# LemonATsu/DANBO-pytorch

Measured on NVIDIA B200. Metric: DANBO render rays/s (fwd+composite), higher is better.
Workload: dtype bf16 (tensor-core MLP, fp32 accumulate); fp32 elsewhere; fp64 box test

## Files before the change

danbo-pytorch_b200/_lib.py:

```python
import ctypes
import os

_HERE = os.path.dirname(os.path.abspath(__file__))
_PATH = os.path.join(_HERE, "libdanbo_b200.so")
_lib = None
ABI_VERSION = 5

c_p = ctypes.c_void_p
c_i = ctypes.c_int
c_f = ctypes.c_float

_SIGNATURES = {
    "danbo_version": [],
    "danbo_nearfar": [c_p, c_i, c_i, c_p, c_i, c_p, c_i, c_i, c_p, c_p, c_i, c_i, c_f, c_f, c_p, c_p, c_p, c_i, c_p, c_p, c_p],
    "danbo_sample_mask": [c_p, c_i, c_i, c_i, c_p, c_p, c_p, c_p, c_p, c_p, c_p, c_i, c_i, c_p, c_p, c_p, c_p, c_i, c_i, c_i, c_p],
    "danbo_field_agg": [c_p, c_i, c_i, c_i, c_p, c_p, c_p, c_p, c_i, c_p, c_p, c_i, c_i, c_p, c_p, c_p, c_p, c_p, c_p, c_p, c_i, c_i, c_i, c_p],
    "danbo_agg_frag_bytes": [],
    "danbo_pair_logits_set_blocks": [c_i],
    "danbo_pack_agg_frags": [c_p, c_p, c_p],
    "danbo_ray_bias": [c_p, c_i, c_i, c_p, c_p, c_i, c_p, c_p, c_p, c_p],
    "danbo_mlp_workspace_bytes": [c_p, c_p, c_p],
    "danbo_mlp_set_pack_empty": [c_i],
    "danbo_mlp_empty_rows": [c_p, c_i, c_p, c_p, c_i, c_p],
    "danbo_mlp_set_cta_pair": [c_i],
    "danbo_graph_net_fwd": [c_p, c_i, c_p, c_p, c_p, c_p],
    "danbo_graph_net_bwd": [c_i, c_p, c_p, c_p, c_p, c_p, c_p],
    "danbo_graph_net_bwd_pose": [c_p, c_i, c_p, c_p, c_p, c_p, c_p],
    "danbo_pose_fwd": [c_p, c_p, c_p, c_p, c_p, c_i, c_p, c_p, c_i, c_i, c_p, c_p, c_f, c_f, c_f, c_p, c_p, c_p, c_p, c_p],
    "danbo_pose_bwd": [c_p, c_p, c_p, c_p, c_p, c_i, c_p, c_p, c_i, c_i, c_p, c_p, c_p, c_p, c_p, c_f, c_f, c_p, c_p, c_p,
                       c_p],
    "danbo_pose_kp2d": [c_p, c_p, c_p, c_i, c_f, c_f, c_p, c_p, c_p],
    "danbo_train_loss": [c_p, c_p, c_p, c_p, c_p, c_p, c_f, c_i, c_i, c_i, c_f, c_f, c_p, c_p, c_p, c_p, c_i, c_f, c_p, c_p, c_f,
                         c_p, c_p, c_p, c_p, c_p, c_p, c_p, c_p],
    "danbo_adam_step": [c_p, c_p, c_p, c_p, ctypes.c_longlong, c_p, c_f, c_f, c_f, c_p, c_i, c_p],
    "danbo_anerf_workspace_bytes": [c_i, c_p, c_p, c_p, c_p],
    "danbo_anerf_pack_weights": [c_p, c_p, c_p, c_p, c_p, c_p, c_p, c_p, c_p, c_p, c_p, c_p, c_p, c_p],
    "danbo_anerf_ray_encode": [c_p, c_i, c_i, c_p, c_i, c_i, c_p, c_p, c_i, c_p, c_p, c_p, c_p],
    "danbo_anerf_embed": [c_p, c_i, c_i, c_p, c_i, c_p, c_i, c_i, c_p, c_p, c_f, c_p, c_p, c_p],
    "danbo_anerf_mlp": [c_p, c_p, c_p, c_p, c_p, c_p, c_i, c_i, c_p, c_i, c_i, c_p, c_p],
    "danbo_anerf_save_bytes": [c_i, c_p],
    "danbo_anerf_mlp_save": [c_p, c_p, c_p, c_p, c_p, c_p, c_i, c_i, c_p, c_i, c_i, c_p, c_p],
# ... 23 lines not shown

EXPORTS = tuple(_SIGNATURES)


def path():
    return _PATH


def load():
    global _lib
    if _lib is None:
        if not os.path.exists(_PATH):
            raise RuntimeError(f"{_PATH} is missing: build it with `python __graft_entry__.py build` "
                               "(there is no CPU fallback for the DANBO hot path)")
        lib = ctypes.CDLL(_PATH)
        for name, argtypes in _SIGNATURES.items():
            fn = getattr(lib, name)
            fn.argtypes = argtypes
            fn.restype = ctypes.c_int
        got = lib.danbo_version()
        if got != ABI_VERSION:
            raise RuntimeError(f"{_PATH} has ABI version {got}, this binding expects {ABI_VERSION}: rebuild it with "
                               "`python __graft_entry__.py build`")
        if os.environ.get("DANBO_PAIR_LOGITS_BLOCKS", ""):
            lib.danbo_pair_logits_set_blocks(int(os.environ["DANBO_PAIR_LOGITS_BLOCKS"]))
        if os.environ.get("DANBO_MLP_CTA_PAIR", "") == "0":
            lib.danbo_mlp_set_cta_pair(0)
        _lib = lib
    return _lib


def check(code, what):
    if code != 0:
        raise RuntimeError(f"{what} failed with code {code}" + (" (cudaError)" if code > 0 else " (invalid argument)"))
```

danbo-pytorch_b200/csrc/field.cu:

```cuda
#include "field_common.cuh"

namespace danbo {

__global__ void nearfar_cyl_kernel(const float* __restrict__ rays, int ray_stride, int n_rays,
                                   const float* __restrict__ pose_cyl, int cyl_stride, int rays_per_pose, int n_poses,
                                   int seg_len, float* __restrict__ near_out, float* __restrict__ far_out,
                                   double* __restrict__ seg_acc ) {
    const int n = blockIdx.x * blockDim.x + threadIdx.x;
    if (n >= n_rays) return;
    const float* r = rays + (size_t)n * ray_stride;
    const float ox = r[0], oz = r[2], dx = r[3], dz = r[5], near = r[6], far = r[7];
    int pose = n / rays_per_pose; if (pose >= n_poses) pose = n_poses - 1;
    const float* c = pose_cyl + (size_t)pose * cyl_stride;
    const float cx = c[0], cz = c[1], rad = c[2];
    const float nx = __fadd_rn(ox, __fmul_rn(dx, near)), nz = __fadd_rn(oz, __fmul_rn(dz, near));
    const float fx = __fadd_rn(ox, __fmul_rn(dx, far)), fz = __fadd_rn(oz, __fmul_rn(dz, far));
    const float ncx = __fsub_rn(cx, nx), ncz = __fsub_rn(cz, nz);
    const float nfx = __fsub_rn(fx, nx), nfz = __fsub_rn(fz, nz);
    const float nf_norm = __fsqrt_rn(__fadd_rn(__fmul_rn(nfx, nfx), __fmul_rn(nfz, nfz)));
    const float scale = __fsqrt_rn(__fadd_rn(__fmul_rn(dx, dx), __fmul_rn(dz, dz)));
    const float cross = __fsub_rn(__fmul_rn(ncx, nfz), __fmul_rn(ncz, nfx));
    const float dist = __fdiv_rn(fabsf(cross), nf_norm);
    const float Q = __fsqrt_rn(__fsub_rn(__fmul_rn(rad, rad), __fmul_rn(dist, dist)));
    const float K = __fdiv_rn(__fadd_rn(__fmul_rn(ncx, nfx), __fmul_rn(ncz, nfz)), nf_norm);
// ... 455 lines not shown
#pragma unroll
                for (int o4 = 0; o4 < 4; ++o4) {
                    const float4 wv = __ldg(w1 + i * (DANBO_AGG_W / 4) + oh * 4 + o4);
#pragma unroll
                    for (int u = 0; u < PP; ++u) {
                        l1[u][4 * o4 + 0] = fmaf(mix[u][i], wv.x, l1[u][4 * o4 + 0]); l1[u][4 * o4 + 1] = fmaf(mix[u][i], wv.y, l1[u][4 * o4 + 1]);
                        l1[u][4 * o4 + 2] = fmaf(mix[u][i], wv.z, l1[u][4 * o4 + 2]); l1[u][4 * o4 + 3] = fmaf(mix[u][i], wv.w, l1[u][4 * o4 + 3]);
                    }
                }
            }
#pragma unroll
            for (int o = 0; o < 16; ++o) {
                const float w2 = __ldg(fc.agg_w2 + j * DANBO_AGG_W + oh * 16 + o);
#pragma unroll
                for (int u = 0; u < PP; ++u) a[u] = fmaf(fmaxf(l1[u][o], 0.f), w2, a[u]);
            }
        }
#pragma unroll
        for (int u = 0; u < PP; ++u)
            if (live[u]) logits[(size_t)id[u] * DANBO_J + j] = a[u];
    }
}

__global__ void __launch_bounds__(128)
field_rows_kernel(const float* __restrict__ rays, int ray_stride, int n_rays, int S, const float* __restrict__ z,
                  const uint32_t* __restrict__ mask, const int* __restrict__ active_ids,
                  const int* __restrict__ active_count, int capacity, const float* __restrict__ pose_skts,
                  const float* __restrict__ pose_vol, int rays_per_pose, int n_poses, FieldConsts fc,
                  const float* __restrict__ logits, uint8_t* __restrict__ xtiles, int* __restrict__ row_ray,
                  float* __restrict__ hbar_out ,
                  __nv_bfloat16* __restrict__ x_rows ,
                  int agg_mode , const int* __restrict__ work) {
    int count = *active_count; if (count > capacity) count = capacity;
    const int total = n_rays * S;
    const float poison = work[DANBO_PAIR_OVERFLOW_WORD] ? __int_as_float(0x7fc00000) : 0.f;
    __shared__ __align__(128) uint8_t stage[4][2][4096];
    const int warp = threadIdx.x >> 5, lane = threadIdx.x & 31;
    int n_flush = 0;
    for (int base = blockIdx.x * blockDim.x; base < count; base += gridDim.x * blockDim.x) {
        if (base + warp * 32 >= count) break;
        const int e = base + threadIdx.x;
        const bool live = e < count;
        const int id = live ? active_ids[e] : total;
        float hbar[DANBO_FEAT];
#pragma unroll
        for (int i = 0; i < DANBO_FEAT; ++i) hbar[i] = 0.f;
        int n;
// ... 32 lines not shown
        if (hbar_out && live) {
            float4* ho = reinterpret_cast<float4*>(hbar_out + (size_t)e * 16);
            ho[0] = make_float4(hbar[0], hbar[1], hbar[2], hbar[3]);   ho[1] = make_float4(hbar[4], hbar[5], hbar[6], hbar[7]);
            ho[2] = make_float4(hbar[8], hbar[9], hbar[10], hbar[11]); ho[3] = make_float4(hbar[12], hbar[13], hbar[14], 0.f);
        }
        float sn[DANBO_FEAT], cs[DANBO_FEAT];
#pragma unroll
        for (int i = 0; i < DANBO_FEAT; ++i) sincosf(hbar[i], &sn[i], &cs[i]);
        const int tile = e >> 7, rr = e & 127;
        uint8_t* xt = xtiles + (size_t)tile * DANBO_X_TILE_BYTES;
        uint32_t pk[4];
#pragma unroll
        for (int col = 0; col < 208; ++col) {
            float v;
            if (col < DANBO_FEAT) v = hbar[col];
            else if (col < DANBO_X_COLS) {
                const int q = col - DANBO_FEAT, rem = q % 30;
                v = rem < DANBO_FEAT ? sn[rem] : cs[rem - DANBO_FEAT];
            } else v = 0.f;
            const uint32_t b = __bfloat16_as_ushort(__float2bfloat16_rn(v));
            if (col & 1) pk[(col & 7) >> 1] |= b << 16; else pk[(col & 7) >> 1] = b;
            if ((col & 7) == 7) {
                const int chunk = (col - 7) >> 6, unit = ((col - 7) & 63) >> 3;
                if (unit == 0) {
                    if (n_flush >= 2) {
                        if (lane == 0) asm volatile("cp.async.bulk.wait_group.read 1;" ::: "memory");
                        __syncwarp();
                    }
                }
                const uint32_t dst = smem_u32(stage[warp][n_flush & 1]) + (uint32_t)(lane * 128 + ((unit ^ (lane & 7)) << 4));
                asm volatile("st.shared.v4.b32 [%0], {%1,%2,%3,%4};" ::"r"(dst), "r"(pk[0]), "r"(pk[1]), "r"(pk[2]), "r"(pk[3]) : "memory");
                if (x_rows && live) *reinterpret_cast<uint4*>(x_rows + (size_t)e * 208 + (col - 7)) = make_uint4(pk[0], pk[1], pk[2], pk[3]);
                if (unit == 7 || col == 207) {
                    asm volatile("fence.proxy.async.shared::cta;" ::: "memory");
                    __syncwarp();
                    if (lane == 0) {
                        uint8_t* gdst = xt + chunk * 16384 + warp * 4096;
                        asm volatile("cp.async.bulk.global.shared::cta.bulk_group [%0], [%1], %2;"
                                     ::"l"(gdst), "r"(smem_u32(stage[warp][n_flush & 1])), "r"(4096u) : "memory");
                        asm volatile("cp.async.bulk.commit_group;" ::: "memory");
                    }
                    ++n_flush;
                }
            }
            if (col >= 44 && (col - 44) % 30 == 0 && col < 194) {
#pragma unroll
                for (int i = 0; i < DANBO_FEAT; ++i) { const float s2 = 2.f * sn[i] * cs[i], c2 = 1.f - 2.f * sn[i] * sn[i]; sn[i] = s2; cs[i] = c2; }
            }
        }
    }
    if (lane == 0) asm volatile("cp.async.bulk.wait_group 0;" ::: "memory");
}

__global__ void __launch_bounds__(128)
code_table_kernel(const float* __restrict__ codes, const float* __restrict__ wv_ray, float* __restrict__ table) {
    const int ci = blockIdx.x, o = threadIdx.x;
    float acc = wv_ray[155 * 128 + o];
    for (int c = 0; c < 128; ++c) acc = fmaf(codes[(size_t)ci * 128 + c], wv_ray[(27 + c) * 128 + o], acc);
    table[ci * 128 + o] = acc;
}

__global__ void __launch_bounds__(128)
ray_bias_kernel(const float* __restrict__ rays, int ray_stride, int n_rays, const int* __restrict__ cam_idx, int n_codes,
                const float* __restrict__ wv_ray ,
                const float* __restrict__ table , float* __restrict__ out ) {
    constexpr int RB = 32, VIN = 27;
// ... 115 lines not shown
    const FieldConsts fc = make_consts(consts);
    const int total = n_rays * S;
    int blocks = (capacity + 255) / 256;
    if (blocks > num_sms * 8) blocks = num_sms * 8;
    pair_bucket_kernel<false><<<blocks, 256, 0, st>>>(mask, active_ids, active_count, capacity, total, pw, pair_capacity, agg_mode);
    DANBO_CHECK_LAUNCH();
    pair_bucket_kernel<true><<<blocks, 256, 0, st>>>(mask, active_ids, active_count, capacity, total, pw, pair_capacity, agg_mode);
    DANBO_CHECK_LAUNCH();
    int pblocks = (pair_capacity / 64 + 24 + 3) / 4;
    if (pblocks > num_sms * 8) pblocks = num_sms * 8;
    const void* agg_frags = consts[10];
    if (agg_frags != nullptr) {
        const int rc = launch_pair_logits_mma(rays, ray_stride, S, z, active_ids, pose_skts, pose_vol, rays_per_pose,
                                              n_poses, fc, pw, pair_capacity, agg_frags, logits, num_sms, st);
        if (rc != 0) return rc;
    } else if (n_poses == 1)
        pair_logits_kernel<true><<<pblocks, 128, 0, st>>>(rays, ray_stride, S, z, active_ids, pose_skts, pose_vol, rays_per_pose,
                                                           n_poses, fc, pw, pair_capacity, logits);
    else
        pair_logits_kernel<false><<<pblocks, 128, 0, st>>>(rays, ray_stride, S, z, active_ids, pose_skts, pose_vol, rays_per_pose,
                                                            n_poses, fc, pw, pair_capacity, logits);
    DANBO_CHECK_LAUNCH();
    int rblocks = (capacity + 127) / 128;
    if (rblocks > num_sms * 16) rblocks = num_sms * 16;
    field_rows_kernel<<<rblocks, 128, 0, st>>>(rays, ray_stride, n_rays, S, z, mask, active_ids, active_count, capacity,
                                                pose_skts, pose_vol, rays_per_pose, n_poses, fc, logits,
                                                (uint8_t*)xtiles, row_ray, hbar_out, (__nv_bfloat16*)x_rows, agg_mode, work);
    DANBO_CHECK_LAUNCH();
    return 0;
}

extern "C" int danbo_ray_bias(const float* rays, int ray_stride, int n_rays, const int* cam_idx, const float* codes,
                              int n_codes, const float* wv_ray, float* table, float* out, void* stream) {
    if (n_rays <= 0) return 0;
    if (!table) return -1;
    code_table_kernel<<<n_codes + 1, 128, 0, (cudaStream_t)stream>>>(codes, wv_ray, table);
    DANBO_CHECK_LAUNCH();
    ray_bias_kernel<<<(n_rays + 31) / 32, 128, 0, (cudaStream_t)stream>>>(rays, ray_stride, n_rays, cam_idx, n_codes, wv_ray,
                                                                       table, out);
    DANBO_CHECK_LAUNCH();
    return 0;
}
```

danbo-pytorch_b200/csrc/field_common.cuh:

```cuda
#pragma once
#include "common.cuh"
#include <math.h>

namespace danbo {

struct FieldConsts {
    const float* align;
    const float* axis_scale;
    const float* agg_w0;
    const float* agg_adjw;
    const float* agg_adj;
    const float* agg_b0;
    const float* agg_w1;
    const float* agg_b1;
    const float* agg_w2;
    const float* agg_b2;
};

static __constant__ uint32_t kNbrMask[DANBO_J] = {
    0x0000000Fu, 0x00000013u, 0x00000025u, 0x00000049u, 0x00000092u, 0x00000124u, 0x00000248u, 0x00000490u,
    0x00000920u, 0x00007240u, 0x00000480u, 0x00000900u, 0x00009200u, 0x00012200u, 0x00024200u, 0x00009000u,
    0x00052000u, 0x000A4000u, 0x00150000u, 0x002A0000u, 0x00540000u, 0x00A80000u, 0x00500000u, 0x00A00000u};

__device__ __forceinline__ void bone_aligned(const float* __restrict__ skt, const float* __restrict__ A,
// ... 12 lines not shown
    t2 = __fadd_rn(fmaf(a2.z, l2, fmaf(a2.y, l1, __fmul_rn(a2.x, l0))), a2.w);
}

__device__ __forceinline__ void bone_coords(const float* __restrict__ skt, const float* __restrict__ A,
                                            const float* __restrict__ scale, float px, float py, float pz,
                                            float& x0, float& x1, float& x2) {
    const float4 r0 = __ldg(reinterpret_cast<const float4*>(skt));
    const float4 r1 = __ldg(reinterpret_cast<const float4*>(skt) + 1);
    const float4 r2 = __ldg(reinterpret_cast<const float4*>(skt) + 2);
    const float l0 = fmaf(r0.z, pz, fmaf(r0.y, py, fmaf(r0.x, px, r0.w)));
    const float l1 = fmaf(r1.z, pz, fmaf(r1.y, py, fmaf(r1.x, px, r1.w)));
    const float l2 = fmaf(r2.z, pz, fmaf(r2.y, py, fmaf(r2.x, px, r2.w)));
    const float4 a0 = __ldg(reinterpret_cast<const float4*>(A));
    const float4 a1 = __ldg(reinterpret_cast<const float4*>(A) + 1);
    const float4 a2 = __ldg(reinterpret_cast<const float4*>(A) + 2);
    const float t0 = __fadd_rn(fmaf(a0.z, l2, fmaf(a0.y, l1, __fmul_rn(a0.x, l0))), a0.w);
    const float t1 = __fadd_rn(fmaf(a1.z, l2, fmaf(a1.y, l1, __fmul_rn(a1.x, l0))), a1.w);
    const float t2 = __fadd_rn(fmaf(a2.z, l2, fmaf(a2.y, l1, __fmul_rn(a2.x, l0))), a2.w);
    x0 = __fdiv_rn(t0, fabsf(__ldg(scale + 0)));
    x1 = __fdiv_rn(t1, fabsf(__ldg(scale + 1)));
    x2 = __fdiv_rn(t2, fabsf(__ldg(scale + 2)));
}

#define DANBO_PAIR_OVERFLOW_WORD 48
struct PairWork {
    int* base;
    __device__ __forceinline__ int* count() const { return base; }
    __device__ __forceinline__ int* cursor() const { return base + 24; }
    __device__ __forceinline__ int* pairs() const { return base + 64; }
};

__device__ __forceinline__ int seg_start(const int* __restrict__ count, int j) {
    int off = 0;
    for (int i = 0; i < j; ++i) off += (count[i] + 31) & ~31;
    return off;
}

template <bool kShared = false>
__device__ __forceinline__ void bone_features(const float* __restrict__ vol_k, float x0, float x1, float x2, float (&h)[DANBO_FEAT]) {
    const float a2 = x0 * x0, b2 = x1 * x1, c2 = x2 * x2;
    const float win = expf(-2.f * (a2 * a2 * a2 + b2 * b2 * b2 + c2 * c2 * c2));
    const float xs[3] = {x0, x1, x2};
#pragma unroll
    for (int a = 0; a < 3; ++a) {
        const float iy = ((xs[a] + 1.f) * (float)DANBO_RES - 1.f) * 0.5f;
        const float fl = floorf(iy);
// ... 30 lines not shown
```

danbo-pytorch_b200/csrc/field_mma.cu:

```cuda
#include "field_common.cuh"

namespace danbo {
namespace aggmma {

constexpr int kHP = 24;
constexpr int kW0Words = DANBO_J * 2 * 4 * 32 * 2;
constexpr int kW1Words = DANBO_J * 2 * 2 * 4 * 32 * 2;

__device__ __forceinline__ uint32_t pack_bf16(__nv_bfloat16 lo_half, __nv_bfloat16 hi_half) {
    __nv_bfloat162 v;
    v.x = lo_half; v.y = hi_half;
    return *reinterpret_cast<uint32_t*>(&v);
}

__device__ __forceinline__ void split(float v, __nv_bfloat16& hi, __nv_bfloat16& lo) {
    hi = __float2bfloat16_rn(v);
    lo = __float2bfloat16_rn(v - __bfloat162float(hi));
}

__device__ __forceinline__ void mma16816(float (&d)[4], const uint32_t (&a)[4], const uint32_t (&b)[2]) {
    asm volatile("mma.sync.aligned.m16n8k16.row.col.f32.bf16.bf16.f32 {%0,%1,%2,%3}, {%4,%5,%6,%7}, {%8,%9}, {%0,%1,%2,%3};\n"
                 : "+f"(d[0]), "+f"(d[1]), "+f"(d[2]), "+f"(d[3])
                 : "r"(a[0]), "r"(a[1]), "r"(a[2]), "r"(a[3]), "r"(b[0]), "r"(b[1]));
}
// ... 6 lines not shown
    int rest = idx < n0 ? idx : idx - n0;
    const int lane = rest & 31; rest >>= 5;
    const int nt = rest & 3; rest >>= 2;
    int s = 0;
    if (idx >= n0) { s = rest & 1; rest >>= 1; }
    const int hl = rest & 1; rest >>= 1;
    const int bone = rest;
    const int g = lane >> 2, t = lane & 3, o = nt * 8 + g;
    float v[4];
#pragma unroll
    for (int e = 0; e < 4; ++e) {
        const int i = s * 16 + 2 * t + (e & 1) + (e >> 1) * 8;
        if (idx < n0) v[e] = i < DANBO_FEAT ? w0[((size_t)bone * DANBO_FEAT + i) * DANBO_AGG_W + o] : 0.f;
        else v[e] = w1[((size_t)bone * DANBO_AGG_W + i) * DANBO_AGG_W + o];
    }
    __nv_bfloat16 h[4], l[4];
#pragma unroll
    for (int e = 0; e < 4; ++e) split(v[e], h[e], l[e]);
    uint32_t* dst = frags + (idx < n0 ? 2 * (size_t)idx : kW0Words + 2 * (size_t)(idx - n0));
    dst[0] = hl ? pack_bf16(l[0], l[1]) : pack_bf16(h[0], h[1]);
    dst[1] = hl ? pack_bf16(l[2], l[3]) : pack_bf16(h[2], h[3]);
}

template <bool kOnePose, int kBlocks>
__global__ void __launch_bounds__(128, kBlocks)
pair_logits_mma_kernel(const float* __restrict__ rays, int ray_stride, int S, const float* __restrict__ z,
                       const int* __restrict__ active_ids, const float* __restrict__ pose_skts,
                       const float* __restrict__ pose_vol, int rays_per_pose, int n_poses, FieldConsts fc, PairWork pw,
                       int pair_capacity, const uint32_t* __restrict__ frags, float* __restrict__ logits) {
    __shared__ __align__(16) float vol_s[kOnePose ? DANBO_J * DANBO_VOL : 4];
    __shared__ __align__(16) __nv_bfloat16 Hs[4][2][32 * kHP];
    __shared__ float outs[4][32];
    const int lane = threadIdx.x & 31, wib = threadIdx.x >> 5;
    const int g = lane >> 2, t = lane & 3;
    if (kOnePose) {
        const float4* src = reinterpret_cast<const float4*>(pose_vol);
        for (int i = threadIdx.x; i < DANBO_J * DANBO_VOL / 4; i += blockDim.x) reinterpret_cast<float4*>(vol_s)[i] = __ldg(src + i);
        __syncthreads();
    }
    const int* cnt = pw.count();
    int n_chunks = 0;
    for (int j = 0; j < DANBO_J; ++j) n_chunks += (cnt[j] + 31) >> 5;
    const int warps = (gridDim.x * blockDim.x) >> 5;
    const uint2* f0 = reinterpret_cast<const uint2*>(frags);
    const uint2* f1 = reinterpret_cast<const uint2*>(frags + kW0Words);
    float b0v[4][2];
#pragma unroll
    for (int nt = 0; nt < 4; ++nt) { b0v[nt][0] = __ldg(fc.agg_b0 + nt * 8 + 2 * t); b0v[nt][1] = __ldg(fc.agg_b0 + nt * 8 + 2 * t + 1); }
    for (int c = (blockIdx.x * blockDim.x + threadIdx.x) >> 5; c < n_chunks; c += warps) {
        int j = 0, first = 0;
        for (;; ++j) { const int nc = (cnt[j] + 31) >> 5; if (c < first + nc) break; first += nc; }
        const int in_seg = (c - first) * 32 + lane;
        const int at = c * 32 + lane;
        const bool live = in_seg < cnt[j] && at < pair_capacity;
        float px = 0.f, py = 0.f, pz = 0.f;
        int id = 0, pose = 0;
        if (live) {
            id = active_ids[pw.pairs()[at]];
            const int n = id / S;
            const float* r = rays + (size_t)n * ray_stride;
            const float zz = z[id];
            px = __fadd_rn(r[0], __fmul_rn(r[3], zz));
            py = __fadd_rn(r[1], __fmul_rn(r[4], zz));
            pz = __fadd_rn(r[2], __fmul_rn(r[5], zz));
            pose = n / rays_per_pose; if (pose >= n_poses) pose = n_poses - 1;
        }
        float acc[2][4][4];
#pragma unroll
        for (int mt = 0; mt < 2; ++mt)
#pragma unroll
            for (int nt = 0; nt < 4; ++nt)
#pragma unroll
                for (int e = 0; e < 4; ++e) acc[mt][nt][e] = 0.f;
        for (uint32_t nb = kNbrMask[j]; nb;) {
            const int k = __ffs(nb) - 1; nb &= nb - 1;
            const float adj = __ldg(fc.agg_adjw + j * DANBO_J + k) * __ldg(fc.agg_adj + j * DANBO_J + k);
            float h[DANBO_FEAT];
            {
                float x0, x1, x2;
                bone_coords(pose_skts + ((size_t)pose * DANBO_J + k) * 16, fc.align + k * 16, fc.axis_scale + k * 3,
                            px, py, pz, x0, x1, x2);
                if (kOnePose) bone_features<true>(vol_s + k * DANBO_VOL, x0, x1, x2, h);
                else bone_features<false>(pose_vol + ((size_t)pose * DANBO_J + k) * DANBO_VOL, x0, x1, x2, h);
            }
            uint32_t wh[8], wl[8];
#pragma unroll
            for (int q = 0; q < 8; ++q) {
                __nv_bfloat16 h0, l0, h1, l1;
                split(live ? h[2 * q] * adj : 0.f, h0, l0);
                if (2 * q + 1 < DANBO_FEAT) split(live ? h[2 * q + 1] * adj : 0.f, h1, l1);
                else { h1 = __float2bfloat16_rn(0.f); l1 = h1; }
                wh[q] = pack_bf16(h0, h1); wl[q] = pack_bf16(l0, l1);
            }
            uint4* rh = reinterpret_cast<uint4*>(Hs[wib][0] + lane * kHP);
            uint4* rl = reinterpret_cast<uint4*>(Hs[wib][1] + lane * kHP);
            rh[0] = make_uint4(wh[0], wh[1], wh[2], wh[3]); rh[1] = make_uint4(wh[4], wh[5], wh[6], wh[7]);
            rl[0] = make_uint4(wl[0], wl[1], wl[2], wl[3]); rl[1] = make_uint4(wl[4], wl[5], wl[6], wl[7]);
            __syncwarp();
            uint32_t a_hi[2][4], a_lo[2][4];
#pragma unroll
            for (int mt = 0; mt < 2; ++mt) {
                const int r0 = mt * 16 + g;
                const uint32_t* Th = reinterpret_cast<const uint32_t*>(Hs[wib][0]);
                const uint32_t* Tl = reinterpret_cast<const uint32_t*>(Hs[wib][1]);
                const int w00 = (r0 * kHP) / 2 + t, w10 = ((r0 + 8) * kHP) / 2 + t;
                a_hi[mt][0] = Th[w00]; a_hi[mt][1] = Th[w10]; a_hi[mt][2] = Th[w00 + 4]; a_hi[mt][3] = Th[w10 + 4];
                a_lo[mt][0] = Tl[w00]; a_lo[mt][1] = Tl[w10]; a_lo[mt][2] = Tl[w00 + 4]; a_lo[mt][3] = Tl[w10 + 4];
            }
#pragma unroll
            for (int nt = 0; nt < 4; ++nt) {
                const uint2 bh = __ldg(f0 + ((k * 2 + 0) * 4 + nt) * 32 + lane);
                const uint2 bl = __ldg(f0 + ((k * 2 + 1) * 4 + nt) * 32 + lane);
                const uint32_t b_hi[2] = {bh.x, bh.y}, b_lo[2] = {bl.x, bl.y};
#pragma unroll
                for (int mt = 0; mt < 2; ++mt) {
                    mma16816(acc[mt][nt], a_hi[mt], b_hi);
                    mma16816(acc[mt][nt], a_lo[mt], b_hi);
                    mma16816(acc[mt][nt], a_hi[mt], b_lo);
                }
            }
            __syncwarp();
        }
        uint32_t m_hi[2][2][4], m_lo[2][2][4];
#pragma unroll
        for (int mt = 0; mt < 2; ++mt)
#pragma unroll
            for (int nt = 0; nt < 4; ++nt) {
                const int s = nt >> 1, half = nt & 1;
                __nv_bfloat16 h0, l0, h1, l1;
                split(fmaxf(acc[mt][nt][0] + b0v[nt][0], 0.f), h0, l0); split(fmaxf(acc[mt][nt][1] + b0v[nt][1], 0.f), h1, l1);
                m_hi[mt][s][half * 2 + 0] = pack_bf16(h0, h1); m_lo[mt][s][half * 2 + 0] = pack_bf16(l0, l1);
                split(fmaxf(acc[mt][nt][2] + b0v[nt][0], 0.f), h0, l0); split(fmaxf(acc[mt][nt][3] + b0v[nt][1], 0.f), h1, l1);
                m_hi[mt][s][half * 2 + 1] = pack_bf16(h0, h1); m_lo[mt][s][half * 2 + 1] = pack_bf16(l0, l1);
            }
#pragma unroll
        for (int mt = 0; mt < 2; ++mt)
#pragma unroll
            for (int nt = 0; nt < 4; ++nt) {
                const float c0 = __ldg(fc.agg_b1 + j * DANBO_AGG_W + nt * 8 + 2 * t), c1 = __ldg(fc.agg_b1 + j * DANBO_AGG_W + nt * 8 + 2 * t + 1);
                acc[mt][nt][0] = c0; acc[mt][nt][1] = c1; acc[mt][nt][2] = c0; acc[mt][nt][3] = c1;
            }
#pragma unroll
        for (int s = 0; s < 2; ++s)
#pragma unroll
            for (int nt = 0; nt < 4; ++nt) {
                const uint2 bh = __ldg(f1 + (((j * 2 + 0) * 2 + s) * 4 + nt) * 32 + lane);
                const uint2 bl = __ldg(f1 + (((j * 2 + 1) * 2 + s) * 4 + nt) * 32 + lane);
                const uint32_t b_hi[2] = {bh.x, bh.y}, b_lo[2] = {bl.x, bl.y};
#pragma unroll
                for (int mt = 0; mt < 2; ++mt) {
                    mma16816(acc[mt][nt], m_hi[mt][s], b_hi);
                    mma16816(acc[mt][nt], m_lo[mt][s], b_hi);
                    mma16816(acc[mt][nt], m_hi[mt][s], b_lo);
                }
            }
        float part[2][2] = {{0.f, 0.f}, {0.f, 0.f}};
#pragma unroll
        for (int nt = 0; nt < 4; ++nt) {
            const float w20 = __ldg(fc.agg_w2 + j * DANBO_AGG_W + nt * 8 + 2 * t), w21 = __ldg(fc.agg_w2 + j * DANBO_AGG_W + nt * 8 + 2 * t + 1);
#pragma unroll
            for (int mt = 0; mt < 2; ++mt) {
                part[mt][0] = fmaf(fmaxf(acc[mt][nt][0], 0.f), w20, fmaf(fmaxf(acc[mt][nt][1], 0.f), w21, part[mt][0]));
                part[mt][1] = fmaf(fmaxf(acc[mt][nt][2], 0.f), w20, fmaf(fmaxf(acc[mt][nt][3], 0.f), w21, part[mt][1]));
            }
        }
        const float b2 = __ldg(fc.agg_b2 + j);
#pragma unroll
        for (int mt = 0; mt < 2; ++mt)
#pragma unroll
            for (int hf = 0; hf < 2; ++hf) {
                float v = part[mt][hf];
                v += __shfl_xor_sync(0xffffffffu, v, 1);
                v += __shfl_xor_sync(0xffffffffu, v, 2);
                if (t == 0) outs[wib][mt * 16 + hf * 8 + g] = v + b2;
            }
        __syncwarp();
        if (live) logits[(size_t)id * DANBO_J + j] = outs[wib][lane];
        __syncwarp();
    }
}

}

static int g_pair_logits_blocks = 4;

int set_pair_logits_blocks(int b) {
    const int old = g_pair_logits_blocks;
    if (b >= 3 && b <= 5) g_pair_logits_blocks = b;
    return old;
}

int launch_pair_logits_mma(const float* rays, int ray_stride, int S, const float* z, const int* active_ids,
                           const float* pose_skts, const float* pose_vol, int rays_per_pose, int n_poses,
                           const FieldConsts& fc, PairWork pw, int pair_capacity, const void* frags, float* logits,
                           int num_sms, cudaStream_t st) {
    const int occ = g_pair_logits_blocks;
    int pblocks = (pair_capacity / 32 + 3) / 4;
    if (pblocks > num_sms * occ) pblocks = num_sms * occ;
    if (pblocks < 1) pblocks = 1;
#define DANBO_PLM_LAUNCH(ONE, OCC) aggmma::pair_logits_mma_kernel<ONE, OCC><<<pblocks, 128, 0, st>>>( \
        rays, ray_stride, S, z, active_ids, pose_skts, pose_vol, rays_per_pose, n_poses, fc, pw, pair_capacity, \
        (const uint32_t*)frags, logits)
    if (n_poses == 1) { if (occ == 3) DANBO_PLM_LAUNCH(true, 3); else if (occ == 4) DANBO_PLM_LAUNCH(true, 4); else DANBO_PLM_LAUNCH(true, 5); }
    else { if (occ == 3) DANBO_PLM_LAUNCH(false, 3); else if (occ == 4) DANBO_PLM_LAUNCH(false, 4); else DANBO_PLM_LAUNCH(false, 5); }
#undef DANBO_PLM_LAUNCH
    DANBO_CHECK_LAUNCH();
    return 0;
}

}

extern "C" int danbo_pair_logits_set_blocks(int blocks) { return danbo::set_pair_logits_blocks(blocks); }

extern "C" int danbo_agg_frag_bytes(void) {
    return (danbo::aggmma::kW0Words + danbo::aggmma::kW1Words) * 4;
}

extern "C" int danbo_pack_agg_frags(const float* const* consts, void* frags, void* stream) {
    if (!consts || !frags) return -1;
    const int n = (danbo::aggmma::kW0Words + danbo::aggmma::kW1Words) / 2;
    danbo::aggmma::pack_frags_kernel<<<(n + 255) / 256, 256, 0, (cudaStream_t)stream>>>(consts[2], consts[6], (uint32_t*)frags);
    DANBO_CHECK_LAUNCH();
    return 0;
}
```

include/danbo_b200.h:

```cpp
#ifndef DANBO_B200_H
#define DANBO_B200_H

#ifdef __cplusplus
extern "C" {
#endif

int danbo_version(void);

int danbo_nearfar(const float* rays, int ray_stride, int n_rays, const float* pose_cyl, int cyl_stride,
                  const float* pose_skts, int rays_per_pose, int n_poses, const float* align, const float* axis_scale,
                  int seg_len, int use_box, float bound, float bound_hi, float* near_out, float* far_out,
                  double* seg_acc, int n_seg, unsigned char* p_valid, unsigned char* v_valid, void* stream);


int danbo_pair_logits_set_blocks(int blocks);

int danbo_agg_frag_bytes(void);
int danbo_pack_agg_frags(const float* const* consts, void* frags, void* stream);

int danbo_sample_mask(const float* rays, int ray_stride, int n_rays, int S, const float* near, const float* far,
                      const float* t_vals, const float* t_rand, const float* z_in, float* z_out,
                      const float* pose_skts, int rays_per_pose, int n_poses, const float* const* consts,
                      unsigned int* mask_out, int* active_ids, int* active_count, int capacity, int append_empty,
                      int lindisp, void* stream);

int danbo_field_agg(const float* rays, int ray_stride, int n_rays, int S, const float* z, const unsigned int* mask,
                    const int* active_ids, const int* active_count, int capacity, const float* pose_skts,
                    const float* pose_vol, int rays_per_pose, int n_poses, const float* const* consts, void* xtiles,
                    int* row_ray, float* logits, float* hbar_out, void* x_rows, int* work, int pair_capacity,
                    int num_sms, int agg_mode, void* stream);

int danbo_mlp_set_pack_empty(int enable);

int danbo_mlp_empty_rows(const float* ray_bias, int n_rays, const float* heads, float* raw_tail, int num_sms, void* stream);

int danbo_ray_bias(const float* rays, int ray_stride, int n_rays, const int* cam_idx, const float* codes, int n_codes,
                   const float* wv_ray, float* table, float* out, void* stream);

// ... 157 lines not shown
```

Baseline: 66.01 million.

## Stage aggregator weights in shared memory and software-pipeline pair loads in logits kernel

The pair-logits MMA kernel becomes a persistent one-block-per-SM kernel with 16 warps. All aggregator MMA fragments and per-bone constants (align, scale, adjacency, biases, skinning transforms) are staged in dynamic shared memory instead of read through __ldg each iteration. Chunk-to-bone lookup now uses a ballot over prefix offsets rather than a serial scan, and pair, id and ray loads are prefetched several chunks ahead. Separately, field_rows_kernel gets a 7-blocks-per-SM launch bound with a matching grid cap, and the last column chunk is written straight to global memory instead of through the bulk-copy staging path. The occupancy tuning knob and its export are removed. Large shared memory use limits occupancy to one block per SM, and the launch bound may force register spills.

```diff
diff --git a/danbo-pytorch_b200/_lib.py b/danbo-pytorch_b200/_lib.py
--- a/danbo-pytorch_b200/_lib.py
+++ b/danbo-pytorch_b200/_lib.py
@@ -16,7 +16,6 @@
     "danbo_sample_mask": [c_p, c_i, c_i, c_i, c_p, c_p, c_p, c_p, c_p, c_p, c_p, c_i, c_i, c_p, c_p, c_p, c_p, c_i, c_i, c_i, c_p],
     "danbo_field_agg": [c_p, c_i, c_i, c_i, c_p, c_p, c_p, c_p, c_i, c_p, c_p, c_i, c_i, c_p, c_p, c_p, c_p, c_p, c_p, c_p, c_i, c_i, c_i, c_p],
     "danbo_agg_frag_bytes": [],
-    "danbo_pair_logits_set_blocks": [c_i],
     "danbo_pack_agg_frags": [c_p, c_p, c_p],
     "danbo_ray_bias": [c_p, c_i, c_i, c_p, c_p, c_i, c_p, c_p, c_p, c_p],
     "danbo_mlp_workspace_bytes": [c_p, c_p, c_p],
@@ -86,8 +85,6 @@
         if got != ABI_VERSION:
             raise RuntimeError(f"{_PATH} has ABI version {got}, this binding expects {ABI_VERSION}: rebuild it with "
                                "`python __graft_entry__.py build`")
-        if os.environ.get("DANBO_PAIR_LOGITS_BLOCKS", ""):
-            lib.danbo_pair_logits_set_blocks(int(os.environ["DANBO_PAIR_LOGITS_BLOCKS"]))
         if os.environ.get("DANBO_MLP_CTA_PAIR", "") == "0":
             lib.danbo_mlp_set_cta_pair(0)
         _lib = lib
diff --git a/danbo-pytorch_b200/csrc/field.cu b/danbo-pytorch_b200/csrc/field.cu
--- a/danbo-pytorch_b200/csrc/field.cu
+++ b/danbo-pytorch_b200/csrc/field.cu
@@ -501,7 +501,8 @@
     }
 }
 
-__global__ void __launch_bounds__(128)
+constexpr int kFieldRowsBlocksPerSm = 7;
+__global__ void __launch_bounds__(128, kFieldRowsBlocksPerSm)
 field_rows_kernel(const float* __restrict__ rays, int ray_stride, int n_rays, int S, const float* __restrict__ z,
                   const uint32_t* __restrict__ mask, const int* __restrict__ active_ids,
                   const int* __restrict__ active_count, int capacity, const float* __restrict__ pose_skts,
@@ -580,26 +581,31 @@
             if (col & 1) pk[(col & 7) >> 1] |= b << 16; else pk[(col & 7) >> 1] = b;
             if ((col & 7) == 7) {
                 const int chunk = (col - 7) >> 6, unit = ((col - 7) & 63) >> 3;
-                if (unit == 0) {
-                    if (n_flush >= 2) {
-                        if (lane == 0) asm volatile("cp.async.bulk.wait_group.read 1;" ::: "memory");
+                if (chunk == 3) {
+                    *reinterpret_cast<uint4*>(xt + 3 * 16384 + rr * 128 + ((unit ^ (rr & 7)) << 4)) =
+                        make_uint4(pk[0], pk[1], pk[2], pk[3]);
+                } else {
+                    if (unit == 0) {
+                        if (n_flush >= 2) {
+                            if (lane == 0) asm volatile("cp.async.bulk.wait_group.read 1;" ::: "memory");
+                            __syncwarp();
+                        }
+                    }
+                    const uint32_t dst = smem_u32(stage[warp][n_flush & 1]) + (uint32_t)(lane * 128 + ((unit ^ (lane & 7)) << 4));
+                    asm volatile("st.shared.v4.b32 [%0], {%1,%2,%3,%4};" ::"r"(dst), "r"(pk[0]), "r"(pk[1]), "r"(pk[2]), "r"(pk[3]) : "memory");
+                    if (unit == 7) {
+                        asm volatile("fence.proxy.async.shared::cta;" ::: "memory");
                         __syncwarp();
+                        if (lane == 0) {
+                            uint8_t* gdst = xt + chunk * 16384 + warp * 4096;
+                            asm volatile("cp.async.bulk.global.shared::cta.bulk_group [%0], [%1], %2;"
+                                         ::"l"(gdst), "r"(smem_u32(stage[warp][n_flush & 1])), "r"(4096u) : "memory");
+                            asm volatile("cp.async.bulk.commit_group;" ::: "memory");
+                        }
+                        ++n_flush;
                     }
                 }
-                const uint32_t dst = smem_u32(stage[warp][n_flush & 1]) + (uint32_t)(lane * 128 + ((unit ^ (lane & 7)) << 4));
-                asm volatile("st.shared.v4.b32 [%0], {%1,%2,%3,%4};" ::"r"(dst), "r"(pk[0]), "r"(pk[1]), "r"(pk[2]), "r"(pk[3]) : "memory");
                 if (x_rows && live) *reinterpret_cast<uint4*>(x_rows + (size_t)e * 208 + (col - 7)) = make_uint4(pk[0], pk[1], pk[2], pk[3]);
-                if (unit == 7 || col == 207) {
-                    asm volatile("fence.proxy.async.shared::cta;" ::: "memory");
-                    __syncwarp();
-                    if (lane == 0) {
-                        uint8_t* gdst = xt + chunk * 16384 + warp * 4096;
-                        asm volatile("cp.async.bulk.global.shared::cta.bulk_group [%0], [%1], %2;"
-                                     ::"l"(gdst), "r"(smem_u32(stage[warp][n_flush & 1])), "r"(4096u) : "memory");
-                        asm volatile("cp.async.bulk.commit_group;" ::: "memory");
-                    }
-                    ++n_flush;
-                }
             }
             if (col >= 44 && (col - 44) % 30 == 0 && col < 194) {
 #pragma unroll
@@ -761,7 +767,7 @@
                                                             n_poses, fc, pw, pair_capacity, logits);
     DANBO_CHECK_LAUNCH();
     int rblocks = (capacity + 127) / 128;
-    if (rblocks > num_sms * 16) rblocks = num_sms * 16;
+    if (rblocks > num_sms * kFieldRowsBlocksPerSm) rblocks = num_sms * kFieldRowsBlocksPerSm;
     field_rows_kernel<<<rblocks, 128, 0, st>>>(rays, ray_stride, n_rays, S, z, mask, active_ids, active_count, capacity,
                                                 pose_skts, pose_vol, rays_per_pose, n_poses, fc, logits,
                                                 (uint8_t*)xtiles, row_ray, hbar_out, (__nv_bfloat16*)x_rows, agg_mode, work);
diff --git a/danbo-pytorch_b200/csrc/field_common.cuh b/danbo-pytorch_b200/csrc/field_common.cuh
--- a/danbo-pytorch_b200/csrc/field_common.cuh
+++ b/danbo-pytorch_b200/csrc/field_common.cuh
@@ -58,6 +58,21 @@
     x2 = __fdiv_rn(t2, fabsf(__ldg(scale + 2)));
 }
 
+__device__ __forceinline__ void bone_coords_staged(const float4* skt, const float4* A, const float* abs_scale,
+                                                   float px, float py, float pz, float& x0, float& x1, float& x2) {
+    const float4 r0 = skt[0], r1 = skt[1], r2 = skt[2];
+    const float l0 = fmaf(r0.z, pz, fmaf(r0.y, py, fmaf(r0.x, px, r0.w)));
+    const float l1 = fmaf(r1.z, pz, fmaf(r1.y, py, fmaf(r1.x, px, r1.w)));
+    const float l2 = fmaf(r2.z, pz, fmaf(r2.y, py, fmaf(r2.x, px, r2.w)));
+    const float4 a0 = A[0], a1 = A[1], a2 = A[2];
+    const float t0 = __fadd_rn(fmaf(a0.z, l2, fmaf(a0.y, l1, __fmul_rn(a0.x, l0))), a0.w);
+    const float t1 = __fadd_rn(fmaf(a1.z, l2, fmaf(a1.y, l1, __fmul_rn(a1.x, l0))), a1.w);
+    const float t2 = __fadd_rn(fmaf(a2.z, l2, fmaf(a2.y, l1, __fmul_rn(a2.x, l0))), a2.w);
+    x0 = __fdiv_rn(t0, abs_scale[0]);
+    x1 = __fdiv_rn(t1, abs_scale[1]);
+    x2 = __fdiv_rn(t2, abs_scale[2]);
+}
+
 #define DANBO_PAIR_OVERFLOW_WORD 48
 struct PairWork {
     int* base;
diff --git a/danbo-pytorch_b200/csrc/field_mma.cu b/danbo-pytorch_b200/csrc/field_mma.cu
--- a/danbo-pytorch_b200/csrc/field_mma.cu
+++ b/danbo-pytorch_b200/csrc/field_mma.cu
@@ -52,48 +52,108 @@
     dst[1] = hl ? pack_bf16(l[2], l[3]) : pack_bf16(h[2], h[3]);
 }
 
-template <bool kOnePose, int kBlocks>
-__global__ void __launch_bounds__(128, kBlocks)
+constexpr int kWarps = 16;
+constexpr int kThreads = kWarps * 32;
+constexpr int kFragBytes = (kW0Words + kW1Words) * 4;
+
+template <bool kOnePose>
+struct alignas(16) PlmShared {
+    uint2 frags[kFragBytes / 8];
+    float vol[kOnePose ? DANBO_J * DANBO_VOL : 4];
+    float4 skt[kOnePose ? DANBO_J * 3 : 1];
+    float4 align[DANBO_J * 3];
+    float scale[DANBO_J * 3];
+    float adj[DANBO_J * DANBO_J];
+    float b1[DANBO_J * DANBO_AGG_W], w2[DANBO_J * DANBO_AGG_W], b2[DANBO_J], b0[DANBO_AGG_W];
+    int first[DANBO_J + 1];
+    int cnt[DANBO_J];
+    alignas(16) __nv_bfloat16 H[kWarps][2][32 * kHP];
+};
+static_assert(sizeof(PlmShared<true>) <= 227 * 1024, "pair_logits_mma_kernel: shared memory over the 227 KB of a block");
+
+__device__ __forceinline__ int chunk_bone(int seg_end, int c) {
+    return __popc(__ballot_sync(0xffffffffu, c >= seg_end));
+}
+
+template <bool kOnePose>
+__global__ void __launch_bounds__(kThreads, 1)
 pair_logits_mma_kernel(const float* __restrict__ rays, int ray_stride, int S, const float* __restrict__ z,
                        const int* __restrict__ active_ids, const float* __restrict__ pose_skts,
                        const float* __restrict__ pose_vol, int rays_per_pose, int n_poses, FieldConsts fc, PairWork pw,
                        int pair_capacity, const uint32_t* __restrict__ frags, float* __restrict__ logits) {
-    __shared__ __align__(16) float vol_s[kOnePose ? DANBO_J * DANBO_VOL : 4];
-    __shared__ __align__(16) __nv_bfloat16 Hs[4][2][32 * kHP];
-    __shared__ float outs[4][32];
-    const int lane = threadIdx.x & 31, wib = threadIdx.x >> 5;
+    extern __shared__ __align__(16) uint8_t smem_raw[];
+    PlmShared<kOnePose>& sm = *reinterpret_cast<PlmShared<kOnePose>*>(smem_raw);
+    const int tid = threadIdx.x, lane = tid & 31, wib = tid >> 5;
     const int g = lane >> 2, t = lane & 3;
+    {
+        const uint4* src = reinterpret_cast<const uint4*>(frags);
+        uint4* dst = reinterpret_cast<uint4*>(sm.frags);
+#pragma unroll 6
+        for (int i = tid; i < kFragBytes / 16; i += kThreads) dst[i] = __ldg(src + i);
+    }
     if (kOnePose) {
         const float4* src = reinterpret_cast<const float4*>(pose_vol);
-        for (int i = threadIdx.x; i < DANBO_J * DANBO_VOL / 4; i += blockDim.x) reinterpret_cast<float4*>(vol_s)[i] = __ldg(src + i);
-        __syncthreads();
-    }
-    const int* cnt = pw.count();
-    int n_chunks = 0;
-    for (int j = 0; j < DANBO_J; ++j) n_chunks += (cnt[j] + 31) >> 5;
-    const int warps = (gridDim.x * blockDim.x) >> 5;
-    const uint2* f0 = reinterpret_cast<const uint2*>(frags);
-    const uint2* f1 = reinterpret_cast<const uint2*>(frags + kW0Words);
+        for (int i = tid; i < DANBO_J * DANBO_VOL / 4; i += kThreads) reinterpret_cast<float4*>(sm.vol)[i] = __ldg(src + i);
+        for (int i = tid; i < DANBO_J * 3; i += kThreads)
+            sm.skt[i] = __ldg(reinterpret_cast<const float4*>(pose_skts) + (i / 3) * 4 + i % 3);
+    }
+    for (int i = tid; i < DANBO_J * 3; i += kThreads) {
+        sm.align[i] = __ldg(reinterpret_cast<const float4*>(fc.align) + (i / 3) * 4 + i % 3);
+        sm.scale[i] = fabsf(__ldg(fc.axis_scale + i));
+    }
+    for (int i = tid; i < DANBO_J * DANBO_J; i += kThreads) sm.adj[i] = __ldg(fc.agg_adjw + i) * __ldg(fc.agg_adj + i);
+    for (int i = tid; i < DANBO_J * DANBO_AGG_W; i += kThreads) { sm.b1[i] = __ldg(fc.agg_b1 + i); sm.w2[i] = __ldg(fc.agg_w2 + i); }
+    if (tid < DANBO_J) sm.b2[tid] = __ldg(fc.agg_b2 + tid);
+    if (tid < DANBO_AGG_W) sm.b0[tid] = __ldg(fc.agg_b0 + tid);
+    if (tid == 0) {
+        const int* cnt = pw.count();
+        int f = 0;
+        for (int j = 0; j < DANBO_J; ++j) { const int n = cnt[j]; sm.first[j] = f; sm.cnt[j] = n; f += (n + 31) >> 5; }
+        sm.first[DANBO_J] = f;
+    }
+    __syncthreads();
+    const int n_chunks = sm.first[DANBO_J];
+    const int seg_end = lane < DANBO_J ? sm.first[lane + 1] : 0x7fffffff;
+    const int stride = gridDim.x * kWarps;
+    const int* pairs = pw.pairs();
+    const uint2* f0 = sm.frags;
+    const uint2* f1 = sm.frags + kW0Words / 2;
     float b0v[4][2];
 #pragma unroll
-    for (int nt = 0; nt < 4; ++nt) { b0v[nt][0] = __ldg(fc.agg_b0 + nt * 8 + 2 * t); b0v[nt][1] = __ldg(fc.agg_b0 + nt * 8 + 2 * t + 1); }
-    for (int c = (blockIdx.x * blockDim.x + threadIdx.x) >> 5; c < n_chunks; c += warps) {
-        int j = 0, first = 0;
-        for (;; ++j) { const int nc = (cnt[j] + 31) >> 5; if (c < first + nc) break; first += nc; }
-        const int in_seg = (c - first) * 32 + lane;
+    for (int nt = 0; nt < 4; ++nt) { b0v[nt][0] = sm.b0[nt * 8 + 2 * t]; b0v[nt][1] = sm.b0[nt * 8 + 2 * t + 1]; }
+    auto pair_of = [&](int c) -> int {
+        if (c >= n_chunks) return -1;
+        const int j = chunk_bone(seg_end, c);
         const int at = c * 32 + lane;
-        const bool live = in_seg < cnt[j] && at < pair_capacity;
+        return ((c - sm.first[j]) * 32 + lane < sm.cnt[j] && at < pair_capacity) ? pairs[at] : -1;
+    };
+    auto point_of = [&](int id, float (&r)[6], float& zz) {
+        if (id < 0) return;
+        const float* rp = rays + (size_t)(id / S) * ray_stride;
+#pragma unroll
+        for (int q = 0; q < 6; ++q) r[q] = rp[q];
+        zz = z[id];
+    };
+    int c = blockIdx.x * kWarps + wib;
+    int p2 = pair_of(c + 2 * stride);
+    int i1 = pair_of(c + stride); i1 = i1 >= 0 ? active_ids[i1] : -1;
+    int id = pair_of(c); id = id >= 0 ? active_ids[id] : -1;
+    float r0[6] = {0.f, 0.f, 0.f, 0.f, 0.f, 0.f}, z0 = 0.f;
+    point_of(id, r0, z0);
+    for (; c < n_chunks; c += stride) {
+        const int p3 = pair_of(c + 3 * stride);
+        const int i2 = p2 >= 0 ? active_ids[p2] : -1;
+        float r1[6] = {0.f, 0.f, 0.f, 0.f, 0.f, 0.f}, z1 = 0.f;
+        point_of(i1, r1, z1);
+        const int j = chunk_bone(seg_end, c);
+        const bool live = id >= 0;
         float px = 0.f, py = 0.f, pz = 0.f;
-        int id = 0, pose = 0;
+        int pose = 0;
         if (live) {
-            id = active_ids[pw.pairs()[at]];
-            const int n = id / S;
-            const float* r = rays + (size_t)n * ray_stride;
-            const float zz = z[id];
-            px = __fadd_rn(r[0], __fmul_rn(r[3], zz));
-            py = __fadd_rn(r[1], __fmul_rn(r[4], zz));
-            pz = __fadd_rn(r[2], __fmul_rn(r[5], zz));
-            pose = n / rays_per_pose; if (pose >= n_poses) pose = n_poses - 1;
+            px = __fadd_rn(r0[0], __fmul_rn(r0[3], z0));
+            py = __fadd_rn(r0[1], __fmul_rn(r0[4], z0));
+            pz = __fadd_rn(r0[2], __fmul_rn(r0[5], z0));
+            pose = (id / S) / rays_per_pose; if (pose >= n_poses) pose = n_poses - 1;
         }
         float acc[2][4][4];
 #pragma unroll
@@ -104,13 +164,14 @@
                 for (int e = 0; e < 4; ++e) acc[mt][nt][e] = 0.f;
         for (uint32_t nb = kNbrMask[j]; nb;) {
             const int k = __ffs(nb) - 1; nb &= nb - 1;
-            const float adj = __ldg(fc.agg_adjw + j * DANBO_J + k) * __ldg(fc.agg_adj + j * DANBO_J + k);
+            const float adj = sm.adj[j * DANBO_J + k];
             float h[DANBO_FEAT];
             {
                 float x0, x1, x2;
-                bone_coords(pose_skts + ((size_t)pose * DANBO_J + k) * 16, fc.align + k * 16, fc.axis_scale + k * 3,
-                            px, py, pz, x0, x1, x2);
-                if (kOnePose) bone_features<true>(vol_s + k * DANBO_VOL, x0, x1, x2, h);
+                const float4* skt = kOnePose ? sm.skt + k * 3
+                                             : reinterpret_cast<const float4*>(pose_skts + ((size_t)pose * DANBO_J + k) * 16);
+                bone_coords_staged(skt, sm.align + k * 3, sm.scale + k * 3, px, py, pz, x0, x1, x2);
+                if (kOnePose) bone_features<true>(sm.vol + k * DANBO_VOL, x0, x1, x2, h);
                 else bone_features<false>(pose_vol + ((size_t)pose * DANBO_J + k) * DANBO_VOL, x0, x1, x2, h);
             }
             uint32_t wh[8], wl[8];
@@ -122,25 +183,25 @@
                 else { h1 = __float2bfloat16_rn(0.f); l1 = h1; }
                 wh[q] = pack_bf16(h0, h1); wl[q] = pack_bf16(l0, l1);
             }
-            uint4* rh = reinterpret_cast<uint4*>(Hs[wib][0] + lane * kHP);
-            uint4* rl = reinterpret_cast<uint4*>(Hs[wib][1] + lane * kHP);
+            uint4* rh = reinterpret_cast<uint4*>(sm.H[wib][0] + lane * kHP);
+            uint4* rl = reinterpret_cast<uint4*>(sm.H[wib][1] + lane * kHP);
             rh[0] = make_uint4(wh[0], wh[1], wh[2], wh[3]); rh[1] = make_uint4(wh[4], wh[5], wh[6], wh[7]);
             rl[0] = make_uint4(wl[0], wl[1], wl[2], wl[3]); rl[1] = make_uint4(wl[4], wl[5], wl[6], wl[7]);
             __syncwarp();
             uint32_t a_hi[2][4], a_lo[2][4];
 #pragma unroll
             for (int mt = 0; mt < 2; ++mt) {
-                const int r0 = mt * 16 + g;
-                const uint32_t* Th = reinterpret_cast<const uint32_t*>(Hs[wib][0]);
-                const uint32_t* Tl = reinterpret_cast<const uint32_t*>(Hs[wib][1]);
-                const int w00 = (r0 * kHP) / 2 + t, w10 = ((r0 + 8) * kHP) / 2 + t;
+                const int r0w = mt * 16 + g;
+                const uint32_t* Th = reinterpret_cast<const uint32_t*>(sm.H[wib][0]);
+                const uint32_t* Tl = reinterpret_cast<const uint32_t*>(sm.H[wib][1]);
+                const int w00 = (r0w * kHP) / 2 + t, w10 = ((r0w + 8) * kHP) / 2 + t;
                 a_hi[mt][0] = Th[w00]; a_hi[mt][1] = Th[w10]; a_hi[mt][2] = Th[w00 + 4]; a_hi[mt][3] = Th[w10 + 4];
                 a_lo[mt][0] = Tl[w00]; a_lo[mt][1] = Tl[w10]; a_lo[mt][2] = Tl[w00 + 4]; a_lo[mt][3] = Tl[w10 + 4];
             }
 #pragma unroll
             for (int nt = 0; nt < 4; ++nt) {
-                const uint2 bh = __ldg(f0 + ((k * 2 + 0) * 4 + nt) * 32 + lane);
-                const uint2 bl = __ldg(f0 + ((k * 2 + 1) * 4 + nt) * 32 + lane);
+                const uint2 bh = f0[((k * 2 + 0) * 4 + nt) * 32 + lane];
+                const uint2 bl = f0[((k * 2 + 1) * 4 + nt) * 32 + lane];
                 const uint32_t b_hi[2] = {bh.x, bh.y}, b_lo[2] = {bl.x, bl.y};
 #pragma unroll
                 for (int mt = 0; mt < 2; ++mt) {
@@ -167,15 +228,15 @@
         for (int mt = 0; mt < 2; ++mt)
 #pragma unroll
             for (int nt = 0; nt < 4; ++nt) {
-                const float c0 = __ldg(fc.agg_b1 + j * DANBO_AGG_W + nt * 8 + 2 * t), c1 = __ldg(fc.agg_b1 + j * DANBO_AGG_W + nt * 8 + 2 * t + 1);
+                const float c0 = sm.b1[j * DANBO_AGG_W + nt * 8 + 2 * t], c1 = sm.b1[j * DANBO_AGG_W + nt * 8 + 2 * t + 1];
                 acc[mt][nt][0] = c0; acc[mt][nt][1] = c1; acc[mt][nt][2] = c0; acc[mt][nt][3] = c1;
             }
 #pragma unroll
         for (int s = 0; s < 2; ++s)
 #pragma unroll
             for (int nt = 0; nt < 4; ++nt) {
-                const uint2 bh = __ldg(f1 + (((j * 2 + 0) * 2 + s) * 4 + nt) * 32 + lane);
-                const uint2 bl = __ldg(f1 + (((j * 2 + 1) * 2 + s) * 4 + nt) * 32 + lane);
+                const uint2 bh = f1[(((j * 2 + 0) * 2 + s) * 4 + nt) * 32 + lane];
+                const uint2 bl = f1[(((j * 2 + 1) * 2 + s) * 4 + nt) * 32 + lane];
                 const uint32_t b_hi[2] = {bh.x, bh.y}, b_lo[2] = {bl.x, bl.y};
 #pragma unroll
                 for (int mt = 0; mt < 2; ++mt) {
@@ -187,14 +248,15 @@
         float part[2][2] = {{0.f, 0.f}, {0.f, 0.f}};
 #pragma unroll
         for (int nt = 0; nt < 4; ++nt) {
-            const float w20 = __ldg(fc.agg_w2 + j * DANBO_AGG_W + nt * 8 + 2 * t), w21 = __ldg(fc.agg_w2 + j * DANBO_AGG_W + nt * 8 + 2 * t + 1);
+            const float w20 = sm.w2[j * DANBO_AGG_W + nt * 8 + 2 * t], w21 = sm.w2[j * DANBO_AGG_W + nt * 8 + 2 * t + 1];
 #pragma unroll
             for (int mt = 0; mt < 2; ++mt) {
                 part[mt][0] = fmaf(fmaxf(acc[mt][nt][0], 0.f), w20, fmaf(fmaxf(acc[mt][nt][1], 0.f), w21, part[mt][0]));
                 part[mt][1] = fmaf(fmaxf(acc[mt][nt][2], 0.f), w20, fmaf(fmaxf(acc[mt][nt][3], 0.f), w21, part[mt][1]));
             }
         }
-        const float b2 = __ldg(fc.agg_b2 + j);
+        const float b2 = sm.b2[j];
+        float* outs = reinterpret_cast<float*>(sm.H[wib][0]);
 #pragma unroll
         for (int mt = 0; mt < 2; ++mt)
 #pragma unroll
@@ -202,45 +264,42 @@
                 float v = part[mt][hf];
                 v += __shfl_xor_sync(0xffffffffu, v, 1);
                 v += __shfl_xor_sync(0xffffffffu, v, 2);
-                if (t == 0) outs[wib][mt * 16 + hf * 8 + g] = v + b2;
+                if (t == 0) outs[mt * 16 + hf * 8 + g] = v + b2;
             }
         __syncwarp();
-        if (live) logits[(size_t)id * DANBO_J + j] = outs[wib][lane];
+        if (live) logits[(size_t)id * DANBO_J + j] = outs[lane];
         __syncwarp();
-    }
-}
-
-}
-
-static int g_pair_logits_blocks = 4;
-
-int set_pair_logits_blocks(int b) {
-    const int old = g_pair_logits_blocks;
-    if (b >= 3 && b <= 5) g_pair_logits_blocks = b;
-    return old;
+        id = i1; i1 = i2; p2 = p3;
+#pragma unroll
+        for (int q = 0; q < 6; ++q) r0[q] = r1[q];
+        z0 = z1;
+    }
+}
+
 }
 
 int launch_pair_logits_mma(const float* rays, int ray_stride, int S, const float* z, const int* active_ids,
                            const float* pose_skts, const float* pose_vol, int rays_per_pose, int n_poses,
                            const FieldConsts& fc, PairWork pw, int pair_capacity, const void* frags, float* logits,
                            int num_sms, cudaStream_t st) {
-    const int occ = g_pair_logits_blocks;
-    int pblocks = (pair_capacity / 32 + 3) / 4;
-    if (pblocks > num_sms * occ) pblocks = num_sms * occ;
+    int pblocks = (pair_capacity / 32 + aggmma::kWarps - 1) / aggmma::kWarps;
+    if (pblocks > num_sms) pblocks = num_sms;
     if (pblocks < 1) pblocks = 1;
-#define DANBO_PLM_LAUNCH(ONE, OCC) aggmma::pair_logits_mma_kernel<ONE, OCC><<<pblocks, 128, 0, st>>>( \
-        rays, ray_stride, S, z, active_ids, pose_skts, pose_vol, rays_per_pose, n_poses, fc, pw, pair_capacity, \
-        (const uint32_t*)frags, logits)
-    if (n_poses == 1) { if (occ == 3) DANBO_PLM_LAUNCH(true, 3); else if (occ == 4) DANBO_PLM_LAUNCH(true, 4); else DANBO_PLM_LAUNCH(true, 5); }
-    else { if (occ == 3) DANBO_PLM_LAUNCH(false, 3); else if (occ == 4) DANBO_PLM_LAUNCH(false, 4); else DANBO_PLM_LAUNCH(false, 5); }
+#define DANBO_PLM_LAUNCH(ONE) do { \
+        auto kern = aggmma::pair_logits_mma_kernel<ONE>; \
+        const int smem = (int)sizeof(aggmma::PlmShared<ONE>); \
+        cudaError_t e = cudaFuncSetAttribute(kern, cudaFuncAttributeMaxDynamicSharedMemorySize, smem); \
+        if (e != cudaSuccess) return (int)e; \
+        kern<<<pblocks, aggmma::kThreads, smem, st>>>(rays, ray_stride, S, z, active_ids, pose_skts, pose_vol, \
+            rays_per_pose, n_poses, fc, pw, pair_capacity, (const uint32_t*)frags, logits); } while (0)
+    if (n_poses == 1) DANBO_PLM_LAUNCH(true);
+    else DANBO_PLM_LAUNCH(false);
 #undef DANBO_PLM_LAUNCH
     DANBO_CHECK_LAUNCH();
     return 0;
 }
 
 }
-
-extern "C" int danbo_pair_logits_set_blocks(int blocks) { return danbo::set_pair_logits_blocks(blocks); }
 
 extern "C" int danbo_agg_frag_bytes(void) {
     return (danbo::aggmma::kW0Words + danbo::aggmma::kW1Words) * 4;
diff --git a/include/danbo_b200.h b/include/danbo_b200.h
--- a/include/danbo_b200.h
+++ b/include/danbo_b200.h
@@ -12,8 +12,6 @@
                   int seg_len, int use_box, float bound, float bound_hi, float* near_out, float* far_out,
                   double* seg_acc, int n_seg, unsigned char* p_valid, unsigned char* v_valid, void* stream);
 
-
-int danbo_pair_logits_set_blocks(int blocks);
 
 int danbo_agg_frag_bytes(void);
 int danbo_pack_agg_frags(const float* const* consts, void* frags, void* stream);
```

Result: no change. 66.17 million, median of 6 (+0.2%).
